# arnaucube/go-snark-study

Hardware: AMD Instinct MI355X
Metric: Groth16 constraints/sec (prove) at 2^20 R1CS (higher is better)
Workload: dtype u32 (9x29-bit Montgomery limbs of the 254-bit BN128 fields)

## Files before the change

### go-snark-study_amd/csrc/msm.h

```cpp
#pragma once
#include <algorithm>
#include <vector>

#include "ec.h"
#include "runtime.h"
#include "tables.h"

namespace gs {

struct PlanBuffers {
  DevBuf digits, hist, totals, offsets, entries, tiles, total;
  DevBuf chunk_bucket, heavy_list, counters;
  DevBuf recs, parts;
};

struct MsmPlan {
  uint32_t n = 0;
  int c = 0, W = 0;
  uint32_t B = 0;
  bool table_free = false;
  uint32_t nbuckets = 0;
  uint32_t chunk = 32;
  uint32_t maxchunks = 0;
  const uint32_t* offsets = nullptr;
  const uint32_t* entries = nullptr;
  const uint32_t* chunk_bucket = nullptr;
  const uint32_t* heavy_list = nullptr;
  const uint32_t* heavy_count = nullptr;
};

constexpr int kMaxWindowBits = 20;
int choose_window_bits(uint32_t n, int forced);
constexpr int kMinFreeWindowBits = 9, kMaxFreeWindowBits = 16;
int choose_window_bits_free(uint32_t n, int forced);

struct MsmBase {
  const BaseTable* table;
  size_t off;
  const uint32_t* points = nullptr;
  size_t npoints = 0;
};

struct LaunchShape { int njobs; bool g2; };
void build_plan(Ctx& c, int slot, const uint32_t* scalars_dev, uint32_t n, MsmPlan& plan, const std::vector<LaunchShape>& users, int cbits = 0,
                bool table_free = false, const uint32_t* term_index = nullptr, uint32_t index_bias = 0);
bool plan_partitions_first(int cbits);
uint32_t finite_mask_dev(Ctx& c, const uint32_t* g1_pts, const uint32_t* g2_pts, uint32_t n, uint32_t* mask_dev);

struct MsmPending {
  int njobs = 0, L = 1, slot = 0, c = 0, W = 0;
  bool table_free = false;
  uint32_t nblk_window = 0;
  uint32_t nblk = 0, n = 0;
  bool g2 = false;
  bool folded = false;
  const void* pinned_slot = nullptr;
  size_t stats_off = 0;
  std::shared_ptr<PhaseTimer> tacc, tker, tred;
};
void msm_enqueue_g1(Ctx& c, const MsmPlan& plan, const std::vector<MsmBase>& bases, int ws_base, int slot, MsmPending& p, hipStream_t tail_stream = nullptr);
void msm_enqueue_g2(Ctx& c, const MsmPlan& plan, const std::vector<MsmBase>& bases, int ws_base, int slot, MsmPending& p, hipStream_t tail_stream = nullptr);
void msm_book_timing(Ctx& c, const MsmPending& p);
void msm_finish_g1(Ctx& c, const MsmPending& p, std::vector<G1Xyzz>& out);
void msm_finish_g2(Ctx& c, const MsmPending& p, std::vector<G2Xyzz>& out);
void msm_run_g1(Ctx& c, const MsmPlan& plan, const std::vector<MsmBase>& bases, std::vector<G1Xyzz>& out);
void msm_run_g2(Ctx& c, const MsmPlan& plan, const std::vector<MsmBase>& bases, std::vector<G2Xyzz>& out);

uint32_t jacobian_to_affine_g1(Ctx& c, const uint32_t* jac_dev, uint32_t n, uint32_t* out_dev, uint32_t* first_bad = nullptr);
uint32_t jacobian_to_affine_g2(Ctx& c, const uint32_t* jac_dev, uint32_t n, uint32_t* out_dev, uint32_t* first_bad = nullptr);
uint32_t upload_jacobian_g1(Ctx& c, const uint64_t* jac_host, uint32_t n, uint32_t* out_dev, uint32_t* first_bad = nullptr);
uint32_t upload_jacobian_g2(Ctx& c, const uint64_t* jac_host, uint32_t n, uint32_t* out_dev, uint32_t* first_bad = nullptr);
void affine_to_jacobian_std_g1(Ctx& c, const uint32_t* aff_dev, uint32_t n, uint32_t* out_dev);
void affine_to_jacobian_std_g2(Ctx& c, const uint32_t* aff_dev, uint32_t n, uint32_t* out_dev);
void fixed_base_g1(Ctx& c, const uint32_t* scalars_dev, uint32_t n, uint32_t* out_dev);
void fixed_base_g2(Ctx& c, const uint32_t* scalars_dev, uint32_t n, uint32_t* out_dev);

G1Affine g1_affine_from_jacobian_std(const uint64_t jac[12]);
G2Affine g2_affine_from_jacobian_std(const uint64_t jac[24]);
bool g1_to_affine_std(const G1Xyzz& p, uint64_t out[8]);
bool g2_to_affine_std(const G2Xyzz& p, uint64_t out[16]);
G1Xyzz g1_mul_scalar(const G1Xyzz& p, const uint64_t k[4]);
G2Xyzz g2_mul_scalar(const G2Xyzz& p, const uint64_t k[4]);
template <class T>
struct HostFixedBase {
  std::vector<Xyzz<T>> win;
  void build(const Affine<T>& p);
  Xyzz<T> mul(const uint64_t k[4]) const;
};
extern template struct HostFixedBase<FqTag>;
extern template struct HostFixedBase<Fq2Tag>;

void fr_canon_words(const uint64_t k[4], uint32_t out[8]);

}
```

### go-snark-study_amd/csrc/msm.hip

```cpp
#include "msm.h"
#include "hostcopy.h"

#include <algorithm>
#include <cmath>
#include <cstdlib>
#include <future>
#include <type_traits>

#include "msm_kernels.h"

namespace gs {

static_assert(sizeof(G1Xyzz) == PointIO<FqTag>::kXyzzWords * 4, "G1 XYZZ must be raw limbs");
static_assert(sizeof(G2Xyzz) == PointIO<Fq2Tag>::kXyzzWords * 4, "G2 XYZZ must be raw limbs");

int choose_window_bits(uint32_t n, int forced) {
  if (forced >= 8 && forced <= kMaxWindowBits) return forced;
  static const double per_bucket = dev_knob_f("GS_WINDOW_COST_BUCKET", 6.0, 0.0, 64.0);
  static const int auto_max = (int)dev_knob("GS_AUTO_MAX_C", 17, 8, kMaxWindowBits);
  int best = 8;
  double best_cost = 1e300;
  for (int c = 8; c <= std::min(kMaxWindowBits, std::max(8, auto_max)); ++c) {
    const int W = 254 / c + 1;
    const double cost = (double)n * W + per_bucket * (double)(1u << (c - 1));
    if (cost < best_cost) { best_cost = cost; best = c; }
  }
  return best;
}

int choose_window_bits_free(uint32_t n, int forced) {
  if (forced) return std::min(kMaxFreeWindowBits, std::max(kMinFreeWindowBits, forced));
  static const double per_bucket = dev_knob_f("GS_WINDOW_COST_BUCKET_FREE", 3.0, 0.0, 64.0);
  int best = kMinFreeWindowBits;
  double best_cost = 1e300;
  for (int c = kMinFreeWindowBits; c <= kMaxFreeWindowBits; ++c) {
    const int W = 254 / c + 1;
    const double cost = (double)W * ((double)n + per_bucket * (double)(1u << (c - 1)));
    if (cost < best_cost) { best_cost = cost; best = c; }
  }
  return best;
}

static void exclusive_scan(Ctx& c, PlanBuffers& pb, const uint32_t* in, uint32_t* out, uint32_t n) {
  const uint32_t ntiles = (n + kScanTile - 1) / kScanTile;
  pb.tiles.ensure((size_t)ntiles * 4);
  pb.total.ensure(4);
  hipLaunchKernelGGL(k_scan_tiles, dim3(ntiles), dim3(kScanBlock), 0, c.stream, in, out, pb.tiles.as<uint32_t>(), n);
  hipLaunchKernelGGL(k_scan_tile_sums, dim3(1), dim3(1024), 0, c.stream, pb.tiles.as<uint32_t>(), ntiles, pb.total.as<uint32_t>());
  hipLaunchKernelGGL(k_scan_add, dim3(ntiles), dim3(kScanBlock), 0, c.stream, out, pb.tiles.as<uint32_t>(), n);
}

struct MsmState {
  PlanBuffers plan_slots[3 * Ctx::kSlots];
  DevBuf upload_scratch;
  DevBuf upload_flag;
  bool lds_attr_set = false;
};
static MsmState& msm_state(Ctx& c) { return c.state<MsmState>(c.msm_state); }

static uint32_t choose_chunk(uint64_t entries, uint32_t nbuckets, const std::vector<LaunchShape>& users) {
  static const int forced = (int)dev_knob("GS_CHUNK", 0, 4, 1024, 4);
  if (forced >= 4 && forced % 4 == 0) return (uint32_t)forced;
  static const int forced_h = (int)dev_knob("GS_CHUNK_H", 0, 4, 1024, 4);
  if (forced_h && users.size() == 1 && users[0].njobs == 1 && !users[0].g2) return (uint32_t)forced_h;
  uint32_t chunk = entries >= (1ull << 27) ? 64u : entries >= (1ull << 23) ? 32u : 16u;
  while (chunk < 1024u && entries / std::max<uint32_t>(nbuckets, 1u) > 32ull * chunk) chunk *= 2;
  return chunk;
}

static uint32_t part_min_ranges() {
  static const uint32_t v = (uint32_t)dev_knob("GS_PART_MIN_R", 4, 2, 64);
  return v;
}
bool plan_partitions_first(int cbits) {
  if (cbits < 1) return false;
  return std::max<uint32_t>(1u, (1u << (cbits - 1)) >> kRangeLog) >= part_min_ranges();
}

uint32_t finite_mask_dev(Ctx& c, const uint32_t* g1_pts, const uint32_t* g2_pts, uint32_t n, uint32_t* mask_dev) {
  const size_t words = ((size_t)n + 31) / 32;
  GS_HIP(hipMemsetAsync(mask_dev, 0, std::max<size_t>(words, 1) * 4, c.stream));
  DevBuf cnt(4);
  GS_HIP(hipMemsetAsync(cnt.p, 0, 4, c.stream));
  if (n) hipLaunchKernelGGL(k_finite_mask, grid1(n), dim3(256), 0, c.stream, g1_pts, (uint32_t)PointIO<FqTag>::kAffineWords, g2_pts,
                            (uint32_t)PointIO<Fq2Tag>::kAffineWords, n, mask_dev, cnt.as<uint32_t>());
  GS_HIP(hipGetLastError());
  uint32_t host = 0;
  GS_HIP(hipMemcpyAsync(&host, cnt.p, 4, hipMemcpyDeviceToHost, c.stream));
  GS_HIP(hipStreamSynchronize(c.stream));
  return host;
}

void build_plan(Ctx& c, int slot, const uint32_t* scalars_dev, uint32_t n, MsmPlan& plan, const std::vector<LaunchShape>& users, int cbits,
                bool table_free, const uint32_t* term_index, uint32_t index_bias) {
  MsmState& ms = msm_state(c);
  PlanBuffers& pb = ms.plan_slots[slot % (3 * Ctx::kSlots)];
  plan.n = n;
  plan.table_free = table_free;
  plan.c = cbits ? cbits : (table_free ? choose_window_bits_free(n, c.window_bits) : choose_window_bits(n, c.window_bits));
  if (table_free && (plan.c < kMinFreeWindowBits || plan.c > kMaxFreeWindowBits))
    throw HipError{hipErrorInvalidValue, "table-free plan outside 9..16 window bits", __LINE__};
  plan.W = 254 / plan.c + 1;
  plan.B = 1u << (plan.c - 1);
  plan.nbuckets = table_free ? (uint32_t)plan.W * plan.B : plan.B;
  plan.chunk = choose_chunk((uint64_t)n * plan.W, plan.nbuckets, users);
  plan.maxchunks = (uint32_t)(((size_t)n * plan.W + plan.chunk - 1) / plan.chunk) + 1;
  const size_t ncount = (size_t)plan.nbuckets + 1;
  PlanParams pp{};
  pp.n = n; pp.c = plan.c; pp.W = plan.W; pp.B = plan.B;
  pp.R = std::max<uint32_t>(1u, plan.B >> kRangeLog);
  pp.tf = table_free ? 1u : 0u;
  {
    const uint32_t want = std::max<uint32_t>(1u, 256u / (plan.W * pp.R));
    const uint32_t by_size = std::max<uint32_t>(1u, (n + 16383u) / 16384u);
    const uint32_t by_mem = std::max<uint32_t>(1u, (uint32_t)((64ull << 20) / ((uint64_t)plan.B * plan.W * 4)));
    pp.S = std::max<uint32_t>(1u, std::min(std::min<uint32_t>(16u, std::max<uint32_t>(want, 1u)), std::min(by_size, by_mem)));
    if (pp.R == 1 && !table_free) pp.S = std::max<uint32_t>(1u, std::min<uint32_t>(16u, by_size));
  }
  pp.slice = (n + pp.S - 1) / pp.S;
  pp.stride = (n + 63u) & ~63u;
  const bool wide = plan_partitions_first(plan.c);
  if (wide && term_index) throw HipError{hipErrorInvalidValue, "plans over a term list cannot be sorted partition-first (plan_partitions_first)", __LINE__};
  const uint32_t nparts = (uint32_t)plan.W * pp.R;
  if (wide && nparts > kMaxParts) throw HipError{hipErrorInvalidValue, "too many (window, range) partitions", __LINE__};
  if (!wide) pb.digits.ensure((size_t)std::max<uint32_t>(pp.stride, 64u) * plan.W * sizeof(digit_t));
  else {
    pb.recs.ensure(std::max<size_t>((size_t)n * plan.W, 1) * 8);
    pb.parts.ensure((size_t)(3 * kMaxParts + 4) * 4);
  }
  pb.hist.ensure((size_t)plan.B * plan.W * pp.S * 4);
  pb.totals.ensure(ncount * 4);
  pb.offsets.ensure(ncount * 4);
  pb.entries.ensure(((size_t)plan.maxchunks + 1) * plan.chunk * 4);
  pb.chunk_bucket.ensure((size_t)plan.maxchunks * 4);
  pb.heavy_list.ensure((size_t)plan.nbuckets * 4);
  pb.counters.ensure(16);
  const size_t lds = (size_t)std::min<uint32_t>(plan.B, kRangeBuckets) * 4;
  static const int sort_block = (int)dev_knob("GS_SORT_BLOCK", kSortBlock, 64, kSortBlock, 64);
  if (!ms.lds_attr_set) {
    GS_HIP(hipFuncSetAttribute(reinterpret_cast<const void*>(k_hist), hipFuncAttributeMaxDynamicSharedMemorySize, 128 * 1024));
    GS_HIP(hipFuncSetAttribute(reinterpret_cast<const void*>(k_scatter), hipFuncAttributeMaxDynamicSharedMemorySize, 128 * 1024));
    GS_HIP(hipFuncSetAttribute(reinterpret_cast<const void*>(k_hist_part), hipFuncAttributeMaxDynamicSharedMemorySize, 128 * 1024));
    GS_HIP(hipFuncSetAttribute(reinterpret_cast<const void*>(k_scatter_part), hipFuncAttributeMaxDynamicSharedMemorySize, 128 * 1024));
    ms.lds_attr_set = true;
  }
  GS_HIP(hipMemsetAsync(pb.totals.as<uint32_t>() + plan.nbuckets, 0, 4, c.stream));
  GS_HIP(hipMemsetAsync(pb.counters.p, 0, 16, c.stream));
  uint32_t* part_count = pb.parts.as<uint32_t>();
  uint32_t* part_base = part_count ? part_count + kMaxParts : nullptr;
  uint32_t* part_cursor = part_count ? part_base + kMaxParts + 4 : nullptr;
  if (n > 0 && wide) {
    GS_HIP(hipMemsetAsync(part_count, 0, (size_t)nparts * 4, c.stream));
    hipLaunchKernelGGL(k_part_count, grid1(n, kPartBlock), dim3(kPartBlock), 0, c.stream, scalars_dev, pp, part_count);
    hipLaunchKernelGGL(k_part_scan, dim3(1), dim3(64), 0, c.stream, part_count, nparts, part_base, part_cursor);
    hipLaunchKernelGGL(k_part_scatter, grid1(n, kPartBlock * kPartPerThread), dim3(kPartBlock), 0, c.stream, scalars_dev, pp, part_base, part_cursor,
                       pb.recs.as<uint2>());
    hipLaunchKernelGGL(k_hist_part, dim3(8 * pp.S * ((nparts + 7) / 8)), dim3(sort_block), lds, c.stream, pb.recs.as<uint2>(), part_base, pp, pb.hist.as<uint32_t>());
    hipLaunchKernelGGL(k_colscan, grid1(plan.B), dim3(256), 0, c.stream, pb.hist.as<uint32_t>(), pp, pb.totals.as<uint32_t>());
  } else if (n > 0) {
    hipLaunchKernelGGL(k_digits, grid1(n), dim3(256), 0, c.stream, scalars_dev, pp, pb.digits.as<digit_t>(), term_index, index_bias);
    hipLaunchKernelGGL(k_hist, dim3(plan.W, pp.S, pp.R), dim3(sort_block), lds, c.stream, pb.digits.as<digit_t>(), pp, pb.hist.as<uint32_t>());
    if (table_free) hipLaunchKernelGGL(k_colscan_windows, grid1(plan.nbuckets), dim3(256), 0, c.stream, pb.hist.as<uint32_t>(), pp, pb.totals.as<uint32_t>());
    else hipLaunchKernelGGL(k_colscan, grid1(plan.B), dim3(256), 0, c.stream, pb.hist.as<uint32_t>(), pp, pb.totals.as<uint32_t>());
  } else {
    GS_HIP(hipMemsetAsync(pb.totals.p, 0, ncount * 4, c.stream));
  }
  exclusive_scan(c, pb, pb.totals.as<uint32_t>(), pb.offsets.as<uint32_t>(), (uint32_t)ncount);
  if (n > 0) {
    if (wide) hipLaunchKernelGGL(k_scatter_part, dim3(8 * pp.S * ((nparts + 7) / 8)), dim3(sort_block), lds, c.stream, pb.recs.as<uint2>(), part_base, pp,
                                 pb.hist.as<uint32_t>(), pb.offsets.as<uint32_t>(), pb.entries.as<uint32_t>());
    else hipLaunchKernelGGL(k_scatter, dim3(plan.W, pp.S, pp.R), dim3(sort_block), lds, c.stream, pb.digits.as<digit_t>(), pp, pb.hist.as<uint32_t>(),
                            pb.offsets.as<uint32_t>(), pb.entries.as<uint32_t>(), term_index, index_bias);
    hipLaunchKernelGGL(k_chunk_map, grid1(plan.nbuckets), dim3(256), 0, c.stream, pb.offsets.as<uint32_t>(), plan.nbuckets, plan.chunk,
                       pb.chunk_bucket.as<uint32_t>(), pb.heavy_list.as<uint32_t>(), pb.counters.as<uint32_t>());
  }
  GS_HIP(hipGetLastError());
  plan.offsets = pb.offsets.as<uint32_t>();
  plan.entries = pb.entries.as<uint32_t>();
  plan.chunk_bucket = pb.chunk_bucket.as<uint32_t>();
  plan.heavy_list = pb.heavy_list.as<uint32_t>();
  plan.heavy_count = pb.counters.as<uint32_t>();
}

template <class T>
static void msm_enqueue(Ctx& c, const MsmPlan& plan, const std::vector<MsmBase>& bases, int ws_base, int slot, MsmPending& p,
                        hipStream_t tail_stream) {
  const int njobs = (int)bases.size();
  p = MsmPending{};
  p.njobs = njobs; p.slot = slot; p.n = plan.n; p.g2 = PointIO<T>::kAffineWords == 32;
  p.c = plan.c; p.W = plan.W;
  if (njobs == 0 || plan.n == 0) { p.njobs = plan.n == 0 ? -njobs : 0; return; }
  if (njobs > kMaxJobs) throw HipError{hipErrorInvalidValue, "too many MSM jobs", __LINE__};
  constexpr size_t pw = PointIO<T>::kXyzzWords;
  constexpr size_t aw = PointIO<T>::kAffineWords;
  static const uint32_t fold_env = (uint32_t)dev_knob("GS_FOLD_MAX", 0, 1, 256);
  const uint32_t fold_max = fold_env ? fold_env : (plan.n >= (1u << 19) ? 32u : 16u);
  static const uint32_t l_min = (uint32_t)dev_knob("GS_REDUCE_L", 4, 1, 32, 1, true);
  int L = (int)std::max<uint32_t>(1u, std::min<uint32_t>(l_min, plan.B / kReduceBlock));
  while (L < 32 && plan.B / ((uint32_t)kReduceBlock * (uint32_t)L) > fold_max) L *= 2;
  uint32_t nblk = (plan.B + kReduceBlock * L - 1) / (kReduceBlock * L);
  if (plan.table_free) {
    L = (int)std::max<uint32_t>(1u, std::min<uint32_t>(16u, plan.B / kReduceBlock));
    p.nblk_window = plan.B / ((uint32_t)kReduceBlock * (uint32_t)L);
    nblk = p.nblk_window * (uint32_t)plan.W;
    p.table_free = true;
  }
  p.L = L; p.nblk = nblk;
  p.folded = !plan.table_free && nblk > fold_max;
  if (p.folded && nblk > (uint32_t)kReduceBlock) throw HipError{hipErrorInvalidValue, "too many reduce workgroups for one fold", __LINE__};
  const size_t pair_bytes = (size_t)njobs * nblk * 2 * pw * 4, final_bytes = (size_t)njobs * pw * 4, stats_bytes = 16;
  const size_t out_bytes = (p.folded ? final_bytes : pair_bytes + final_bytes) + stats_bytes;
  if (out_bytes > Ctx::kPinnedBytes) throw HipError{hipErrorInvalidValue, "MSM result staging too small", __LINE__};
  p.stats_off = out_bytes - stats_bytes;
  AccJobs jobs{};
  DevBuf& outb = c.ws_out[ws_base % Ctx::kWsSets];
  outb.ensure(pair_bytes + final_bytes + stats_bytes);
  uint32_t* finals = outb.as<uint32_t>() + pair_bytes / 4;
  uint32_t* stats = finals + final_bytes / 4;
  for (int j = 0; j < njobs; ++j) {
    const BaseTable* t = bases[j].table;
    const uint32_t* points = nullptr;
    uint32_t row_stride = 0;
    if (plan.table_free) {
      if (!bases[j].points || bases[j].off + plan.n > bases[j].npoints)
        throw HipError{hipErrorInvalidValue, "MSM base array does not cover the plan", __LINE__};
      points = bases[j].points + bases[j].off * aw;
    } else {
      if (!t || t->c != plan.c || !t->rows.p || bases[j].off + plan.n > t->n)
        throw HipError{hipErrorInvalidValue, "MSM base table does not match the plan", __LINE__};
      points = t->rows.as<uint32_t>() + bases[j].off * aw;
      row_stride = (uint32_t)t->n;
    }
    DevBuf& bk = c.ws_buckets[(ws_base + j) % Ctx::kWsSets];
    DevBuf& mg = c.ws_chunks[(ws_base + j) % Ctx::kWsSets];
    DevBuf& pt = c.ws_partials[(ws_base + j) % Ctx::kWsSets];
    bk.ensure((size_t)plan.nbuckets * pw * 4);
    mg.ensure((size_t)plan.nbuckets * pw * 4);
    pt.ensure((size_t)plan.maxchunks * 2 * pw * 4);
    jobs.j[j] = AccJob{points, row_stride, bk.as<uint32_t>(), pt.as<uint32_t>(),
                       pt.as<uint32_t>() + (size_t)plan.maxchunks * pw, mg.as<uint32_t>(),
                       outb.as<uint32_t>() + (size_t)j * nblk * 2 * pw, finals + (size_t)j * pw};
  }
  p.tacc = std::make_shared<PhaseTimer>(c.stream);
  p.tker = std::make_shared<PhaseTimer>(c.stream);
  hipLaunchKernelGGL(k_bucket_accumulate<T>, dim3((plan.maxchunks + kAccBlock - 1) / kAccBlock, njobs), dim3(kAccBlock), 0, c.stream,
                     jobs, plan.offsets, plan.entries, plan.chunk_bucket, plan.nbuckets, plan.chunk);
  p.tker->stop();
  p.tacc->stop();
  hipStream_t ts = tail_stream ? tail_stream : c.stream;
  if (ts != c.stream) {
    hipEvent_t ev;
    GS_HIP(hipEventCreateWithFlags(&ev, hipEventDisableTiming));
    GS_HIP(hipEventRecord(ev, c.stream));
    GS_HIP(hipStreamWaitEvent(ts, ev, 0));
    GS_HIP(hipEventDestroy(ev));
  }
  p.tred = std::make_shared<PhaseTimer>(ts);
  static const long alone_below_log2 = dev_knob("GS_TAIL_ALONE_LOG2", 19, 0, 32);
  const bool alone = plan.n < (1ull << alone_below_log2);
  auto launch_tails = [&](auto alone_tag) {
    constexpr bool kAlone = decltype(alone_tag)::value;
    hipLaunchKernelGGL((k_heavy_combine<T, kAlone>), dim3(64, njobs), dim3(kHeavyBlock), 0, ts,
                       jobs, plan.offsets, plan.heavy_list, plan.heavy_count, plan.chunk);
    hipLaunchKernelGGL((k_heavy_finish<T, kAlone>), dim3(16, njobs), dim3(kHeavyBlock), 0, ts,
// ... 226 lines not shown
```

### go-snark-study_amd/csrc/msm_kernels.h

```cpp
#pragma once
#include <hip/hip_runtime.h>
#include <stdint.h>

#include "ec.h"
#include "point_io.h"

namespace gs {

struct PlanParams {
  uint32_t n;
  int c;
  int W;
  uint32_t B;
  uint32_t S;
  uint32_t slice;
  uint32_t stride;
  uint32_t R;
  uint32_t tf;
};
constexpr uint32_t kRangeLog = 15;
constexpr uint32_t kRangeBuckets = 1u << kRangeLog;

GS_HD int32_t next_digit(const uint32_t (&k)[8], const PlanParams& pp, int w, uint32_t& carry) {
  uint32_t raw = scalar_bits(k, w * pp.c, pp.c) + carry;
  if (raw > pp.B) { carry = 1; return (int32_t)raw - (int32_t)(2u * pp.B); }
  carry = 0;
  return (int32_t)raw;
}

using digit_t = uint32_t;
__global__ void __launch_bounds__(256) k_digits(const uint32_t* __restrict__ scalars, PlanParams pp, digit_t* __restrict__ digits,
                                                 const uint32_t* __restrict__ term_index, uint32_t index_bias) {
  wave_priority<GS_PRIO_PLAN>();
  const uint32_t i = blockIdx.x * blockDim.x + threadIdx.x;
  if (i >= pp.n) return;
  const uint32_t src = term_index ? term_index[i] - index_bias : i;
  uint32_t k[8];
  const uint4* s4 = reinterpret_cast<const uint4*>(scalars + (size_t)src * 8);
  uint4 lo = s4[0], hi = s4[1];
  k[0] = lo.x; k[1] = lo.y; k[2] = lo.z; k[3] = lo.w; k[4] = hi.x; k[5] = hi.y; k[6] = hi.z; k[7] = hi.w;
  scalar_canon(k);
  uint32_t carry = 0;
  for (int w = 0; w < pp.W; ++w) {
    const int32_t d = next_digit(k, pp, w, carry);
    digits[(size_t)w * pp.stride + i] = (digit_t)(d + (int32_t)pp.B - 1);
  }
}

__global__ void __launch_bounds__(256) k_finite_mask(const uint32_t* __restrict__ a, uint32_t wa, const uint32_t* __restrict__ b, uint32_t wb, uint32_t n,
                                                      uint32_t* __restrict__ mask, uint32_t* __restrict__ count) {
  const uint32_t i = blockIdx.x * blockDim.x + threadIdx.x;
  bool finite = false;
  if (i < n) {
    uint32_t acc = 0;
    if (a) for (uint32_t k = 0; k < wa; ++k) acc |= a[(size_t)i * wa + k];
    if (b) for (uint32_t k = 0; k < wb; ++k) acc |= b[(size_t)i * wb + k];
    finite = acc != 0;
  }
  if (finite) { atomicOr(&mask[i >> 5], 1u << (i & 31u)); atomicAdd(count, 1u); }
}

constexpr int kSortBlock = 1024;

__global__ void __launch_bounds__(kSortBlock) k_hist(const digit_t* __restrict__ digits, PlanParams pp, uint32_t* __restrict__ hist) {
  wave_priority<GS_PRIO_PLAN>();
  extern __shared__ uint32_t sh[];
  const uint32_t w = blockIdx.x, s = blockIdx.y, r = blockIdx.z;
  const uint32_t nb = min(pp.B, kRangeBuckets), base = r << kRangeLog;
  for (uint32_t b = threadIdx.x; b < nb; b += blockDim.x) sh[b] = 0;
  __syncthreads();
  const uint32_t lo = s * pp.slice, hi = min(pp.n, lo + pp.slice);
  const digit_t* row = digits + (size_t)w * pp.stride;
  const int32_t zero = (int32_t)pp.B - 1;
  for (uint32_t i = lo + threadIdx.x; i < hi; i += blockDim.x) {
    const int32_t d = (int32_t)row[i] - zero;
    if (d != 0) {
      const uint32_t b = (uint32_t)(d < 0 ? -d : d) - 1u;
      if ((b >> kRangeLog) == r) atomicAdd(&sh[b - base], 1u);
    }
  }
  __syncthreads();
  uint32_t* out = hist + ((size_t)w * pp.S + s) * pp.B + base;
  for (uint32_t b = threadIdx.x; b < nb; b += blockDim.x) out[b] = sh[b];
}

__global__ void __launch_bounds__(256) k_colscan(uint32_t* __restrict__ hist, PlanParams pp, uint32_t* __restrict__ totals) {
  wave_priority<GS_PRIO_PLAN>();
  const uint32_t b = blockIdx.x * blockDim.x + threadIdx.x;
  if (b >= pp.B) return;
  uint32_t* col = hist + b;
  const uint32_t nq = (uint32_t)pp.W * pp.S;
  uint32_t run = 0;
  for (uint32_t q = 0; q < nq; ++q) { const uint32_t t = col[(size_t)q * pp.B]; col[(size_t)q * pp.B] = run; run += t; }
  totals[b] = run;
}

__global__ void __launch_bounds__(256) k_colscan_windows(uint32_t* __restrict__ hist, PlanParams pp, uint32_t* __restrict__ totals) {
  wave_priority<GS_PRIO_PLAN>();
  const uint32_t i = blockIdx.x * blockDim.x + threadIdx.x;
  if (i >= (uint32_t)pp.W * pp.B) return;
  const uint32_t w = i / pp.B, b = i % pp.B;
  uint32_t* col = hist + (size_t)w * pp.S * pp.B + b;
  uint32_t run = 0;
  for (uint32_t q = 0; q < pp.S; ++q) { const uint32_t t = col[(size_t)q * pp.B]; col[(size_t)q * pp.B] = run; run += t; }
  totals[i] = run;
}

__global__ void __launch_bounds__(kSortBlock) k_scatter(const digit_t* __restrict__ digits, PlanParams pp, const uint32_t* __restrict__ hist,
                                                         const uint32_t* __restrict__ offsets, uint32_t* __restrict__ entries,
                                                         const uint32_t* __restrict__ term_index, uint32_t index_bias) {
  wave_priority<GS_PRIO_PLAN>();
  extern __shared__ uint32_t sh[];
  const uint32_t w = blockIdx.x, s = blockIdx.y, r = blockIdx.z;
  const uint32_t nb = min(pp.B, kRangeBuckets), base = r << kRangeLog;
  const uint32_t* pre = hist + ((size_t)w * pp.S + s) * pp.B + base;
  const uint32_t* off = offsets + (pp.tf ? (size_t)w * pp.B : (size_t)0);
  for (uint32_t b = threadIdx.x; b < nb; b += blockDim.x) sh[b] = off[base + b] + pre[b];
  __syncthreads();
  const uint32_t lo = s * pp.slice, hi = min(pp.n, lo + pp.slice);
  const digit_t* row = digits + (size_t)w * pp.stride;
  const int32_t zero = (int32_t)pp.B - 1;
  for (uint32_t i = lo + threadIdx.x; i < hi; i += blockDim.x) {
    const int32_t d = (int32_t)row[i] - zero;
    if (d != 0) {
      const uint32_t b = (uint32_t)(d < 0 ? -d : d) - 1u;
      if ((b >> kRangeLog) == r) {
        const uint32_t pos = atomicAdd(&sh[b - base], 1u);
        const uint32_t id = term_index ? term_index[i] - index_bias : i;
        entries[pos] = id | (w << kWindowShift) | (d < 0 ? kSignBit : 0u);
      }
    }
  }
}

constexpr int kPartBlock = 256;
constexpr int kPartPerThread = 4;
constexpr uint32_t kMaxParts = 512;

GS_HD void load_scalar_canon(const uint32_t* __restrict__ scalars, uint32_t i, uint32_t (&k)[8]) {
  const uint4* s4 = reinterpret_cast<const uint4*>(scalars + (size_t)i * 8);
  const uint4 lo = s4[0], hi = s4[1];
  k[0] = lo.x; k[1] = lo.y; k[2] = lo.z; k[3] = lo.w; k[4] = hi.x; k[5] = hi.y; k[6] = hi.z; k[7] = hi.w;
  scalar_canon(k);
}

__global__ void __launch_bounds__(kPartBlock) k_part_count(const uint32_t* __restrict__ scalars, PlanParams pp, uint32_t* __restrict__ part_count) {
  wave_priority<GS_PRIO_PLAN>();
  __shared__ uint32_t cnt[kMaxParts];
  const uint32_t nparts = (uint32_t)pp.W * pp.R;
  for (uint32_t t = threadIdx.x; t < nparts; t += kPartBlock) cnt[t] = 0;
  __syncthreads();
  const uint32_t i = blockIdx.x * kPartBlock + threadIdx.x;
  if (i < pp.n) {
    uint32_t k[8];
    load_scalar_canon(scalars, i, k);
    uint32_t carry = 0;
    for (int w = 0; w < pp.W; ++w) {
      const int32_t d = next_digit(k, pp, w, carry);
      if (d != 0) atomicAdd(&cnt[(uint32_t)w * pp.R + (((uint32_t)(d < 0 ? -d : d) - 1u) >> kRangeLog)], 1u);
    }
  }
  __syncthreads();
  for (uint32_t t = threadIdx.x; t < nparts; t += kPartBlock) if (cnt[t]) atomicAdd(&part_count[t], cnt[t]);
}

__global__ void __launch_bounds__(64) k_part_scan(uint32_t* __restrict__ part_count, uint32_t nparts, uint32_t* __restrict__ part_base,
                                                    uint32_t* __restrict__ part_cursor) {
  wave_priority<GS_PRIO_PLAN>();
  if (blockIdx.x != 0 || threadIdx.x != 0) return;
  uint32_t run = 0;
  for (uint32_t t = 0; t < nparts; ++t) { part_base[t] = run; run += part_count[t]; part_cursor[t] = 0; part_count[t] = 0; }
  part_base[nparts] = run;
}

__global__ void __launch_bounds__(kPartBlock) k_part_scatter(const uint32_t* __restrict__ scalars, PlanParams pp, const uint32_t* __restrict__ part_base,
                                                              uint32_t* __restrict__ part_cursor, uint2* __restrict__ recs) {
  wave_priority<GS_PRIO_PLAN>();
  __shared__ uint32_t cnt[kMaxParts];
  const uint32_t nparts = (uint32_t)pp.W * pp.R;
  for (uint32_t t = threadIdx.x; t < nparts; t += kPartBlock) cnt[t] = 0;
  __syncthreads();
  const uint32_t first = blockIdx.x * (kPartBlock * kPartPerThread);
  for (int j = 0; j < kPartPerThread; ++j) {
    const uint32_t i = first + j * kPartBlock + threadIdx.x;
    if (i >= pp.n) break;
    uint32_t k[8];
    load_scalar_canon(scalars, i, k);
    uint32_t carry = 0;
    for (int w = 0; w < pp.W; ++w) {
      const int32_t d = next_digit(k, pp, w, carry);
      if (d != 0) atomicAdd(&cnt[(uint32_t)w * pp.R + (((uint32_t)(d < 0 ? -d : d) - 1u) >> kRangeLog)], 1u);
    }
  }
  __syncthreads();
  for (uint32_t t = threadIdx.x; t < nparts; t += kPartBlock) {
    const uint32_t mine = cnt[t];
    cnt[t] = part_base[t] + (mine ? atomicAdd(&part_cursor[t], mine) : 0u);
  }
  __syncthreads();
  for (int j = 0; j < kPartPerThread; ++j) {
    const uint32_t i = first + j * kPartBlock + threadIdx.x;
    if (i >= pp.n) break;
    uint32_t k[8];
    load_scalar_canon(scalars, i, k);
    uint32_t carry = 0;
    for (int w = 0; w < pp.W; ++w) {
      const int32_t d = next_digit(k, pp, w, carry);
      if (d != 0) {
        const uint32_t b = (uint32_t)(d < 0 ? -d : d) - 1u;
        const uint32_t pos = atomicAdd(&cnt[(uint32_t)w * pp.R + (b >> kRangeLog)], 1u);
        recs[pos] = make_uint2(i | (d < 0 ? kSignBit : 0u), b);
      }
    }
  }
}

GS_HD bool part_of_block(uint32_t id, const PlanParams& pp, uint32_t& w, uint32_t& r, uint32_t& s) {
  const uint32_t xcd = id & 7u, j = id >> 3;
  const uint32_t p = xcd + 8u * (j / pp.S);
  s = j % pp.S;
// ... 33 lines not shown
  uint32_t w, r, s;
  if (!part_of_block(blockIdx.x, pp, w, r, s)) return;
  const uint32_t base = r << kRangeLog;
  const uint32_t* pre = hist + ((size_t)w * pp.S + s) * pp.B + base;
  for (uint32_t b = threadIdx.x; b < kRangeBuckets; b += blockDim.x) sh[b] = offsets[base + b] + pre[b];
  __syncthreads();
  uint32_t lo, hi;
  part_slice(part_base, pp, w, r, s, lo, hi);
  for (uint32_t e = lo + threadIdx.x; e < hi; e += blockDim.x) {
    const uint2 rec = recs[e];
    entries[atomicAdd(&sh[rec.y - base], 1u)] = rec.x | (w << kWindowShift);
  }
}

constexpr int kScanBlock = 256;
constexpr int kScanPerThread = 8;
constexpr int kScanTile = kScanBlock * kScanPerThread;

__global__ void __launch_bounds__(kScanBlock) k_scan_tiles(const uint32_t* __restrict__ in, uint32_t* __restrict__ out,
                                                            uint32_t* __restrict__ tile_sums, uint32_t n) {
  wave_priority<GS_PRIO_PLAN>();
  __shared__ uint32_t sh[kScanBlock];
  const uint32_t base = blockIdx.x * kScanTile + threadIdx.x * kScanPerThread;
  uint32_t v[kScanPerThread], sum = 0;
#pragma unroll
  for (int j = 0; j < kScanPerThread; ++j) { v[j] = (base + j < n) ? in[base + j] : 0u; sum += v[j]; }
  sh[threadIdx.x] = sum;
  __syncthreads();
  for (int off = 1; off < kScanBlock; off <<= 1) {
    uint32_t t = (threadIdx.x >= (uint32_t)off) ? sh[threadIdx.x - off] : 0u;
    __syncthreads();
    sh[threadIdx.x] += t;
    __syncthreads();
  }
  uint32_t run = sh[threadIdx.x] - sum;
#pragma unroll
  for (int j = 0; j < kScanPerThread; ++j) { if (base + j < n) out[base + j] = run; run += v[j]; }
  if (threadIdx.x == kScanBlock - 1) tile_sums[blockIdx.x] = sh[threadIdx.x];
}

__global__ void __launch_bounds__(1024) k_scan_tile_sums(uint32_t* __restrict__ tile_sums, uint32_t ntiles, uint32_t* __restrict__ total) {
  wave_priority<GS_PRIO_PLAN>();
  __shared__ uint32_t sh[1024];
  const uint32_t per = (ntiles + 1023u) / 1024u;
  const uint32_t b0 = threadIdx.x * per;
  uint32_t sum = 0;
  for (uint32_t j = 0; j < per; ++j) if (b0 + j < ntiles) sum += tile_sums[b0 + j];
  sh[threadIdx.x] = sum;
  __syncthreads();
  for (int off = 1; off < 1024; off <<= 1) {
    uint32_t t = (threadIdx.x >= (uint32_t)off) ? sh[threadIdx.x - off] : 0u;
    __syncthreads();
    sh[threadIdx.x] += t;
    __syncthreads();
  }
  uint32_t run = sh[threadIdx.x] - sum;
  for (uint32_t j = 0; j < per; ++j) if (b0 + j < ntiles) { uint32_t t = tile_sums[b0 + j]; tile_sums[b0 + j] = run; run += t; }
  if (threadIdx.x == 1023) *total = sh[1023];
}

__global__ void __launch_bounds__(kScanBlock) k_scan_add(uint32_t* __restrict__ out, const uint32_t* __restrict__ tile_sums, uint32_t n) {
  wave_priority<GS_PRIO_PLAN>();
  const uint32_t base = blockIdx.x * kScanTile + threadIdx.x * kScanPerThread;
  const uint32_t add = tile_sums[blockIdx.x];
#pragma unroll
  for (int j = 0; j < kScanPerThread; ++j) if (base + j < n) out[base + j] += add;
}

constexpr uint32_t kHeavySpan = 64;

__global__ void __launch_bounds__(256) k_chunk_map(const uint32_t* __restrict__ offsets, uint32_t nbuckets, uint32_t chunk,
                                                    uint32_t* __restrict__ chunk_bucket, uint32_t* __restrict__ heavy_list,
                                                    uint32_t* __restrict__ heavy_count) {
  wave_priority<GS_PRIO_PLAN>();
  const uint32_t b = blockIdx.x * blockDim.x + threadIdx.x;
  if (b >= nbuckets) return;
  const uint32_t o0 = offsets[b], o1 = offsets[b + 1];
  if (o1 == o0) return;
  const uint32_t t0 = (o0 + chunk - 1) / chunk, t1 = (o1 + chunk - 1) / chunk;
  for (uint32_t t = t0; t < t1; ++t) chunk_bucket[t] = b;
  if ((o1 - 1) / chunk - o0 / chunk > kHeavySpan) {
    heavy_list[atomicAdd(heavy_count, 1u)] = b;
  }
}

struct AccJob {
  const uint32_t* table;
  uint32_t row_stride;
  uint32_t* buckets;
  uint32_t* heads;
  uint32_t* tails;
  uint32_t* merged;
  uint32_t* out;
  uint32_t* final_out;
};
constexpr int kMaxJobs = 8;
struct AccJobs { AccJob j[kMaxJobs]; };

template <class T> struct AccTuning;
#ifndef GS_G1_WAVES
#define GS_G1_WAVES 3
#endif
#ifndef GS_G1_PREFETCH
#define GS_G1_PREFETCH 1
#endif
#ifndef GS_G2_TOUCH
#define GS_G2_TOUCH 0
#endif
template <> struct AccTuning<FqTag> { static constexpr int kMinWaves = GS_G1_WAVES; static constexpr bool kRegisterPrefetch = GS_G1_PREFETCH != 0; static constexpr bool kTouch = true; };
#ifndef GS_G2_WAVES
#define GS_G2_WAVES 2
#endif
#ifndef GS_G2_PREFETCH
#define GS_G2_PREFETCH 0
#endif
template <> struct AccTuning<Fq2Tag> { static constexpr int kMinWaves = GS_G2_WAVES; static constexpr bool kRegisterPrefetch = GS_G2_PREFETCH != 0; static constexpr bool kTouch = GS_G2_TOUCH != 0; };

#ifndef GS_ACC_BLOCK
#define GS_ACC_BLOCK 256
#endif
constexpr int kAccBlock = GS_ACC_BLOCK;
template <class T>
__global__ void __launch_bounds__(kAccBlock, AccTuning<T>::kMinWaves) k_bucket_accumulate(AccJobs jobs, const uint32_t* __restrict__ offsets,
                                                            const uint32_t* __restrict__ entries,
                                                            const uint32_t* __restrict__ chunk_bucket, uint32_t nbuckets, uint32_t chunk) {
  constexpr int pw = PointIO<T>::kXyzzWords;
  constexpr int aw = PointIO<T>::kAffineWords;
  const uint32_t t = blockIdx.x * blockDim.x + threadIdx.x;
  const uint32_t total = offsets[nbuckets];
  const uint32_t beg = t * chunk;
  if (beg >= total) return;
  const uint32_t end = min(beg + chunk, total);
  const AccJob job = jobs.j[blockIdx.y];
  uint32_t b = chunk_bucket[t];
  uint32_t bend = offsets[b + 1];
  bool started_before = offsets[b] < beg;
  constexpr bool kTight = GS_PAIR != 0 && T::kWords != 8;
  using Acc = std::conditional_t<kTight, XyzzAcc<T>, Xyzz<T>>;
  auto acc_inf = [] { if constexpr (kTight) return xyzz_acc_inf<T>(); else return xyzz_inf<T>(); };
  auto acc_store = [](uint32_t* p, const Acc& a) { if constexpr (kTight) store_xyzz<T>(p, to_xyzz(a)); else store_xyzz<T>(p, a); };
  Acc acc = acc_inf();
  const uint4* e4 = reinterpret_cast<const uint4*>(entries + beg);
  constexpr bool kPre = AccTuning<T>::kRegisterPrefetch;
  uint4 q = e4[0];
  uint32_t v = q.x;
  uint32_t nb = b;
  const uint32_t* np = job.table + ((size_t)((v >> kWindowShift) & 31u) * job.row_stride + (v & kIndexMask)) * aw;
  RawAffine<T> nextp;
  uint32_t touch = 0;
  if constexpr (kPre) nextp = load_raw_affine<T>(np);
  for (uint32_t e = beg; e < end; ++e) {
    const uint32_t cur = v;
    const uint32_t* cp = np;
    RawAffine<T> curp;
    if constexpr (kPre) curp = nextp;
    if (e >= bend) {
      acc_store((started_before ? job.heads + (size_t)t * pw : job.buckets + (size_t)b * pw), acc);
      started_before = false;
      acc = acc_inf();
      b = nb; bend = offsets[b + 1];
    }
    if (e + 1 < end) {
      const uint32_t k = (e + 1 - beg) & 3u;
      if (k == 0) q = e4[(e + 1 - beg) >> 2];
      v = k == 0 ? q.x : k == 1 ? q.y : k == 2 ? q.z : q.w;
      uint32_t nbend = offsets[nb + 1];
// ... 313 lines not shown
```

Baseline: 128.9 million.

## Add packed partition-first bucket sort for MSM plans at mid window sizes

Adds a third plan-building path for window sizes 15-17 with up to 2^22 terms. Scalars are counted and scattered into (range, window) partitions as packed 32-bit records (sign, low bucket bits, term index). Per-slice histograms, a column scan and a final scatter then produce the bucket-sorted entries. This replaces the digit-matrix path for these sizes to cut the memory traffic of writing and re-reading a full digit matrix. The cost is more kernel launches, recomputing digits twice, and a larger shared partition table (kMaxParts raised to 2048).

```diff
diff --git a/go-snark-study_amd/csrc/msm.h b/go-snark-study_amd/csrc/msm.h
--- a/go-snark-study_amd/csrc/msm.h
+++ b/go-snark-study_amd/csrc/msm.h
@@ -12,6 +12,7 @@
   DevBuf digits, hist, totals, offsets, entries, tiles, total;
   DevBuf chunk_bucket, heavy_list, counters;
   DevBuf recs, parts;
+  DevBuf pack_tables;
 };
 
 struct MsmPlan {
diff --git a/go-snark-study_amd/csrc/msm.hip b/go-snark-study_amd/csrc/msm.hip
--- a/go-snark-study_amd/csrc/msm.hip
+++ b/go-snark-study_amd/csrc/msm.hip
@@ -68,14 +68,19 @@
   return chunk;
 }
 
+enum class PlanSort { kMatrix, kWide, kPacked };
+constexpr uint32_t kPackedMinTerms = 1;
 static uint32_t part_min_ranges() {
   static const uint32_t v = (uint32_t)dev_knob("GS_PART_MIN_R", 4, 2, 64);
   return v;
 }
-bool plan_partitions_first(int cbits) {
-  if (cbits < 1) return false;
-  return std::max<uint32_t>(1u, (1u << (cbits - 1)) >> kRangeLog) >= part_min_ranges();
-}
+static PlanSort plan_sort(int cbits, uint32_t n, bool table_free, bool term_list) {
+  if (cbits < 1) return PlanSort::kMatrix;
+  if (std::max<uint32_t>(1u, (1u << (cbits - 1)) >> kRangeLog) >= part_min_ranges()) return PlanSort::kWide;
+  if (!table_free && !term_list && n >= kPackedMinTerms && pack_serves(n, cbits)) return PlanSort::kPacked;
+  return PlanSort::kMatrix;
+}
+bool plan_partitions_first(int cbits) { return plan_sort(cbits, 0, false, true) != PlanSort::kMatrix; }
 
 uint32_t finite_mask_dev(Ctx& c, const uint32_t* g1_pts, const uint32_t* g2_pts, uint32_t n, uint32_t* mask_dev) {
   const size_t words = ((size_t)n + 31) / 32;
@@ -89,6 +94,52 @@
   GS_HIP(hipMemcpyAsync(&host, cnt.p, 4, hipMemcpyDeviceToHost, c.stream));
   GS_HIP(hipStreamSynchronize(c.stream));
   return host;
+}
+
+static void publish_plan(MsmPlan& plan, PlanBuffers& pb) {
+  plan.offsets = pb.offsets.as<uint32_t>();
+  plan.entries = pb.entries.as<uint32_t>();
+  plan.chunk_bucket = pb.chunk_bucket.as<uint32_t>();
+  plan.heavy_list = pb.heavy_list.as<uint32_t>();
+  plan.heavy_count = pb.counters.as<uint32_t>();
+}
+
+static void build_plan_packed(Ctx& c, PlanBuffers& pb, const uint32_t* scalars_dev, MsmPlan& plan) {
+  PackParams P{};
+  P.n = plan.n; P.c = plan.c; P.W = plan.W; P.B = plan.B; P.chunk = plan.chunk;
+  P.L = pack_layout(plan.n, plan.c);
+  if (P.L.nparts > kMaxParts || P.L.NR > kPackMaxRanges || P.L.rb < (uint32_t)kPackMinRangeBits || (P.L.NR << P.L.rb) != plan.B)
+    throw HipError{hipErrorInvalidValue, "packed plan layout out of range", __LINE__};
+  const size_t nrec = (size_t)plan.n * plan.W;
+  pb.recs.ensure(nrec * 4);
+  const size_t table_words = 3 * (size_t)kMaxParts + 4 + 2 * (size_t)kPackMaxRanges + 4 + 8;
+  pb.pack_tables.ensure(table_words * 4);
+  pb.hist.ensure(((size_t)P.L.max_slices + 1) << P.L.rb << 2);
+  pb.offsets.ensure(((size_t)plan.nbuckets + 1) * 4);
+  pb.entries.ensure(((size_t)plan.maxchunks + 1) * plan.chunk * 4);
+  pb.chunk_bucket.ensure((size_t)plan.maxchunks * 4);
+  pb.heavy_list.ensure((size_t)plan.nbuckets * 4);
+  pb.counters.ensure(16);
+  PackTables T{};
+  T.count = pb.pack_tables.as<uint32_t>();
+  T.base = T.count + kMaxParts;
+  T.cursor = T.base + kMaxParts + 4;
+  T.xfirst = T.cursor + kMaxParts;
+  T.sbase = T.xfirst + kPackMaxRanges;
+  T.xtotal = T.sbase + kPackMaxRanges + 4;
+  GS_HIP(hipMemsetAsync(T.count, 0, (size_t)P.L.nparts * 4, c.stream));
+  GS_HIP(hipMemsetAsync(pb.counters.p, 0, 16, c.stream));
+  const uint32_t tiles = (plan.n + P.L.tile - 1) / P.L.tile, slice_grid = 8u * P.L.max_xslices;
+  hipLaunchKernelGGL(k_pack_count, dim3(tiles), dim3(kPackBlock), 0, c.stream, scalars_dev, P, T);
+  hipLaunchKernelGGL(k_pack_scan, dim3(1), dim3(kPackBlock), 0, c.stream, P, T);
+  hipLaunchKernelGGL(k_pack_scatter, dim3(tiles), dim3(kPackBlock), 0, c.stream, scalars_dev, P, T, pb.recs.as<uint32_t>());
+  hipLaunchKernelGGL(k_pack_hist, dim3(slice_grid), dim3(kPackBlock), 0, c.stream, pb.recs.as<uint32_t>(), P, T, pb.hist.as<uint32_t>());
+  hipLaunchKernelGGL(k_pack_offsets, dim3(P.L.NR), dim3(1u << P.L.rb), 0, c.stream, P, T, pb.hist.as<uint32_t>(), pb.offsets.as<uint32_t>(),
+                     pb.chunk_bucket.as<uint32_t>(), pb.heavy_list.as<uint32_t>(), pb.counters.as<uint32_t>());
+  hipLaunchKernelGGL(k_pack_entries, dim3(slice_grid), dim3(kPackBlock), 0, c.stream, pb.recs.as<uint32_t>(), P, T, pb.hist.as<uint32_t>(),
+                     pb.offsets.as<uint32_t>(), pb.entries.as<uint32_t>());
+  GS_HIP(hipGetLastError());
+  publish_plan(plan, pb);
 }
 
 void build_plan(Ctx& c, int slot, const uint32_t* scalars_dev, uint32_t n, MsmPlan& plan, const std::vector<LaunchShape>& users, int cbits,
@@ -119,7 +170,9 @@
   }
   pp.slice = (n + pp.S - 1) / pp.S;
   pp.stride = (n + 63u) & ~63u;
-  const bool wide = plan_partitions_first(plan.c);
+  const PlanSort sort = plan_sort(plan.c, n, table_free, term_index != nullptr);
+  if (sort == PlanSort::kPacked) { build_plan_packed(c, pb, scalars_dev, plan); return; }
+  const bool wide = sort == PlanSort::kWide;
   if (wide && term_index) throw HipError{hipErrorInvalidValue, "plans over a term list cannot be sorted partition-first (plan_partitions_first)", __LINE__};
   const uint32_t nparts = (uint32_t)plan.W * pp.R;
   if (wide && nparts > kMaxParts) throw HipError{hipErrorInvalidValue, "too many (window, range) partitions", __LINE__};
@@ -175,11 +228,7 @@
                        pb.chunk_bucket.as<uint32_t>(), pb.heavy_list.as<uint32_t>(), pb.counters.as<uint32_t>());
   }
   GS_HIP(hipGetLastError());
-  plan.offsets = pb.offsets.as<uint32_t>();
-  plan.entries = pb.entries.as<uint32_t>();
-  plan.chunk_bucket = pb.chunk_bucket.as<uint32_t>();
-  plan.heavy_list = pb.heavy_list.as<uint32_t>();
-  plan.heavy_count = pb.counters.as<uint32_t>();
+  publish_plan(plan, pb);
 }
 
 template <class T>
diff --git a/go-snark-study_amd/csrc/msm_kernels.h b/go-snark-study_amd/csrc/msm_kernels.h
--- a/go-snark-study_amd/csrc/msm_kernels.h
+++ b/go-snark-study_amd/csrc/msm_kernels.h
@@ -3,6 +3,7 @@
 #include <stdint.h>
 
 #include "ec.h"
+#include "plan_layout.h"
 #include "point_io.h"
 
 namespace gs {
@@ -21,12 +22,13 @@
 constexpr uint32_t kRangeLog = 15;
 constexpr uint32_t kRangeBuckets = 1u << kRangeLog;
 
-GS_HD int32_t next_digit(const uint32_t (&k)[8], const PlanParams& pp, int w, uint32_t& carry) {
-  uint32_t raw = scalar_bits(k, w * pp.c, pp.c) + carry;
-  if (raw > pp.B) { carry = 1; return (int32_t)raw - (int32_t)(2u * pp.B); }
+GS_HD int32_t digit_of(const uint32_t (&k)[8], int c, uint32_t B, int w, uint32_t& carry) {
+  uint32_t raw = scalar_bits(k, w * c, c) + carry;
+  if (raw > B) { carry = 1; return (int32_t)raw - (int32_t)(2u * B); }
   carry = 0;
   return (int32_t)raw;
 }
+GS_HD int32_t next_digit(const uint32_t (&k)[8], const PlanParams& pp, int w, uint32_t& carry) { return digit_of(k, pp.c, pp.B, w, carry); }
 
 using digit_t = uint32_t;
 __global__ void __launch_bounds__(256) k_digits(const uint32_t* __restrict__ scalars, PlanParams pp, digit_t* __restrict__ digits,
@@ -135,7 +137,7 @@
 
 constexpr int kPartBlock = 256;
 constexpr int kPartPerThread = 4;
-constexpr uint32_t kMaxParts = 512;
+constexpr uint32_t kMaxParts = 2048;
 
 GS_HD void load_scalar_canon(const uint32_t* __restrict__ scalars, uint32_t i, uint32_t (&k)[8]) {
   const uint4* s4 = reinterpret_cast<const uint4*>(scalars + (size_t)i * 8);
@@ -335,6 +337,214 @@
   if ((o1 - 1) / chunk - o0 / chunk > kHeavySpan) {
     heavy_list[atomicAdd(heavy_count, 1u)] = b;
   }
+}
+
+constexpr int kPackBlock = 256;
+struct PackParams {
+  uint32_t n;
+  int c, W;
+  uint32_t B;
+  uint32_t chunk;
+  PackLayout L;
+};
+struct PackTables {
+  uint32_t* count;
+  uint32_t* base;
+  uint32_t* cursor;
+  uint32_t* xfirst;
+  uint32_t* sbase;
+  uint32_t* xtotal;
+};
+
+__device__ __forceinline__ void pack_count_tile(const uint32_t* __restrict__ scalars, const PackParams& P, uint32_t* cnt) {
+  const uint32_t first = blockIdx.x * P.L.tile;
+  for (uint32_t j = 0; j < P.L.tile; j += kPackBlock) {
+    const uint32_t i = first + j + threadIdx.x;
+    if (i >= P.n) break;
+    uint32_t k[8];
+    load_scalar_canon(scalars, i, k);
+    uint32_t carry = 0;
+    for (int w = 0; w < P.W; ++w) {
+      const int32_t d = digit_of(k, P.c, P.B, w, carry);
+      if (d != 0) atomicAdd(&cnt[pack_partition(pack_bucket_range((uint32_t)(d < 0 ? -d : d) - 1u, P.L.rb), (uint32_t)w, (uint32_t)P.W)], 1u);
+    }
+  }
+}
+
+__global__ void __launch_bounds__(kPackBlock) k_pack_count(const uint32_t* __restrict__ scalars, PackParams P, PackTables T) {
+  wave_priority<GS_PRIO_PLAN>();
+  __shared__ uint32_t cnt[kMaxParts];
+  for (uint32_t t = threadIdx.x; t < P.L.nparts; t += kPackBlock) cnt[t] = 0;
+  __syncthreads();
+  pack_count_tile(scalars, P, cnt);
+  __syncthreads();
+  for (uint32_t t = threadIdx.x; t < P.L.nparts; t += kPackBlock) if (cnt[t]) atomicAdd(&T.count[t], cnt[t]);
+}
+
+__global__ void __launch_bounds__(kPackBlock) k_pack_scan(PackParams P, PackTables T) {
+  wave_priority<GS_PRIO_PLAN>();
+  static_assert(kMaxParts <= 8 * kPackBlock, "k_pack_scan: eight partitions per thread");
+  __shared__ uint32_t sb[kMaxParts + 1];
+  __shared__ uint32_t ssum[kPackBlock];
+  __shared__ uint32_t snsl[kPackMaxRanges];
+  const uint32_t nparts = P.L.nparts, per = (nparts + kPackBlock - 1u) / kPackBlock, t0 = threadIdx.x * per;
+  uint32_t v[8], sum = 0;
+#pragma unroll
+  for (uint32_t j = 0; j < 8; ++j) { v[j] = (j < per && t0 + j < nparts) ? T.count[t0 + j] : 0u; sum += v[j]; }
+  ssum[threadIdx.x] = sum;
+  __syncthreads();
+  for (int off = 1; off < kPackBlock; off <<= 1) {
+    const uint32_t t = (threadIdx.x >= (uint32_t)off) ? ssum[threadIdx.x - off] : 0u;
+    __syncthreads();
+    ssum[threadIdx.x] += t;
+    __syncthreads();
+  }
+  uint32_t run = ssum[threadIdx.x] - sum;
+#pragma unroll
+  for (uint32_t j = 0; j < 8; ++j)
+    if (j < per && t0 + j < nparts) { sb[t0 + j] = run; T.base[t0 + j] = run; T.cursor[t0 + j] = 0; run += v[j]; }
+  if (threadIdx.x == kPackBlock - 1) { sb[nparts] = ssum[kPackBlock - 1]; T.base[nparts] = ssum[kPackBlock - 1]; }
+  __syncthreads();
+  const uint32_t NR = P.L.NR, W = (uint32_t)P.W;
+  for (uint32_t r = threadIdx.x; r < NR; r += kPackBlock) snsl[r] = pack_slices(sb[(r + 1u) * W] - sb[r * W], P.L.slice_len);
+  __syncthreads();
+  for (uint32_t r = threadIdx.x; r < NR; r += kPackBlock) {
+    uint32_t xf = 0, sbv = 0;
+    for (uint32_t q = r & 7u; q < r; q += 8u) xf += snsl[q];
+    for (uint32_t q = 0; q < r; ++q) sbv += snsl[q];
+    T.xfirst[r] = xf;
+    T.sbase[r] = sbv;
+    if (r == NR - 1u) T.sbase[NR] = sbv + snsl[r];
+  }
+  if (threadIdx.x < 8u) {
+    uint32_t xt = 0;
+    for (uint32_t q = threadIdx.x; q < NR; q += 8u) xt += snsl[q];
+    T.xtotal[threadIdx.x] = xt;
+  }
+}
+
+__global__ void __launch_bounds__(kPackBlock) k_pack_scatter(const uint32_t* __restrict__ scalars, PackParams P, PackTables T, uint32_t* __restrict__ recs) {
+  wave_priority<GS_PRIO_PLAN>();
+  __shared__ uint32_t cnt[kMaxParts];
+  for (uint32_t t = threadIdx.x; t < P.L.nparts; t += kPackBlock) cnt[t] = 0;
+  __syncthreads();
+  pack_count_tile(scalars, P, cnt);
+  __syncthreads();
+  for (uint32_t t = threadIdx.x; t < P.L.nparts; t += kPackBlock) {
+    const uint32_t mine = cnt[t];
+    cnt[t] = T.base[t] + (mine ? atomicAdd(&T.cursor[t], mine) : 0u);
+  }
+  __syncthreads();
+  const uint32_t first = blockIdx.x * P.L.tile;
+  for (uint32_t j = 0; j < P.L.tile; j += kPackBlock) {
+    const uint32_t i = first + j + threadIdx.x;
+    if (i >= P.n) break;
+    uint32_t k[8];
+    load_scalar_canon(scalars, i, k);
+    uint32_t carry = 0;
+    for (int w = 0; w < P.W; ++w) {
+      const int32_t d = digit_of(k, P.c, P.B, w, carry);
+      if (d != 0) {
+        const uint32_t b = (uint32_t)(d < 0 ? -d : d) - 1u;
+        const uint32_t pos = atomicAdd(&cnt[pack_partition(pack_bucket_range(b, P.L.rb), (uint32_t)w, (uint32_t)P.W)], 1u);
+        recs[pos] = pack_record(d < 0, pack_bucket_low(b, P.L.rb), i, P.L.rb);
+      }
+    }
+  }
+}
+
+__device__ __forceinline__ bool pack_block_slice(const PackParams& P, const PackTables& T, uint32_t& r, uint32_t& row, uint32_t& lo, uint32_t& hi) {
+  const uint32_t x = blockIdx.x & 7u, j = blockIdx.x >> 3;
+  if (x >= P.L.NR || j >= T.xtotal[x]) return false;
+  r = x;
+  for (uint32_t q = x + 8u; q < P.L.NR && T.xfirst[q] <= j; q += 8u) r = q;
+  const uint32_t s = j - T.xfirst[r];
+  row = T.sbase[r] + s;
+  pack_slice_bounds(T.base[r * (uint32_t)P.W], T.base[(r + 1u) * (uint32_t)P.W], s, P.L.slice_len, lo, hi);
+  return true;
+}
+
+__global__ void __launch_bounds__(kPackBlock) k_pack_hist(const uint32_t* __restrict__ recs, PackParams P, PackTables T, uint32_t* __restrict__ hist) {
+  wave_priority<GS_PRIO_PLAN>();
+  __shared__ uint32_t sh[1u << kPackMaxRangeBits];
+  uint32_t r, row, lo, hi;
+  if (!pack_block_slice(P, T, r, row, lo, hi)) return;
+  const uint32_t rb = P.L.rb, nb = 1u << rb;
+  for (uint32_t b = threadIdx.x; b < nb; b += kPackBlock) sh[b] = 0;
+  __syncthreads();
+  uint32_t e = lo + threadIdx.x;
+  for (; e + 3u * kPackBlock < hi; e += 4u * kPackBlock) {
+    const uint32_t r0 = recs[e], r1 = recs[e + kPackBlock], r2 = recs[e + 2u * kPackBlock], r3 = recs[e + 3u * kPackBlock];
+    atomicAdd(&sh[record_bucket_low(r0, rb)], 1u);
+    atomicAdd(&sh[record_bucket_low(r1, rb)], 1u);
+    atomicAdd(&sh[record_bucket_low(r2, rb)], 1u);
+    atomicAdd(&sh[record_bucket_low(r3, rb)], 1u);
+  }
+  for (; e < hi; e += kPackBlock) atomicAdd(&sh[record_bucket_low(recs[e], rb)], 1u);
+  __syncthreads();
+  uint32_t* out = hist + (size_t)row * nb;
+  for (uint32_t b = threadIdx.x; b < nb; b += kPackBlock) out[b] = sh[b];
+}
+
+__global__ void __launch_bounds__(1 << kPackMaxRangeBits) k_pack_offsets(PackParams P, PackTables T, uint32_t* __restrict__ hist, uint32_t* __restrict__ offsets,
+                                                                         uint32_t* __restrict__ chunk_bucket, uint32_t* __restrict__ heavy_list,
+                                                                         uint32_t* __restrict__ heavy_count) {
+  wave_priority<GS_PRIO_PLAN>();
+  __shared__ uint32_t sc[1u << kPackMaxRangeBits];
+  const uint32_t r = blockIdx.x, b = threadIdx.x, nb = 1u << P.L.rb;
+  const uint32_t row0 = T.sbase[r], row1 = T.sbase[r + 1u];
+  uint32_t* col = hist + (size_t)row0 * nb + b;
+  uint32_t run = 0, row = row0;
+  for (; row + 4u <= row1; row += 4u, col += 4u * (size_t)nb) {
+    const uint32_t t0 = col[0], t1 = col[nb], t2 = col[2u * (size_t)nb], t3 = col[3u * (size_t)nb];
+    col[0] = run; col[nb] = run + t0; col[2u * (size_t)nb] = run + t0 + t1; col[3u * (size_t)nb] = run + t0 + t1 + t2;
+    run += t0 + t1 + t2 + t3;
+  }
+  for (; row < row1; ++row, col += nb) { const uint32_t t = col[0]; col[0] = run; run += t; }
+  sc[b] = run;
+  __syncthreads();
+  for (uint32_t off = 1; off < nb; off <<= 1) {
+    const uint32_t t = (b >= off) ? sc[b - off] : 0u;
+    __syncthreads();
+    sc[b] += t;
+    __syncthreads();
+  }
+  const uint32_t o0 = T.base[r * (uint32_t)P.W] + sc[b] - run, o1 = o0 + run;
+  const uint32_t bucket = pack_bucket_of(r, b, P.L.rb);
+  offsets[bucket] = o0;
+  if (bucket == P.B - 1u) offsets[P.B] = o1;
+  if (o1 == o0) return;
+  const uint32_t chunk = P.chunk;
+  const uint32_t c0 = (o0 + chunk - 1u) / chunk, c1 = (o1 + chunk - 1u) / chunk;
+  for (uint32_t t = c0; t < c1; ++t) chunk_bucket[t] = bucket;
+  if ((o1 - 1u) / chunk - o0 / chunk > kHeavySpan) heavy_list[atomicAdd(heavy_count, 1u)] = bucket;
+}
+
+__global__ void __launch_bounds__(kPackBlock) k_pack_entries(const uint32_t* __restrict__ recs, PackParams P, PackTables T, const uint32_t* __restrict__ hist,
+                                                              const uint32_t* __restrict__ offsets, uint32_t* __restrict__ entries) {
+  wave_priority<GS_PRIO_PLAN>();
+  __shared__ uint32_t sh[1u << kPackMaxRangeBits];
+  __shared__ uint32_t wb[32];
+  uint32_t r, row, lo, hi;
+  if (!pack_block_slice(P, T, r, row, lo, hi)) return;
+  const uint32_t rb = P.L.rb, nb = 1u << rb, W = (uint32_t)P.W;
+  const uint32_t* pre = hist + (size_t)row * nb;
+  const uint32_t* off = offsets + ((size_t)r << rb);
+  for (uint32_t b = threadIdx.x; b < nb; b += kPackBlock) sh[b] = off[b] + pre[b];
+  if (threadIdx.x <= W) wb[threadIdx.x] = T.base[r * W + threadIdx.x];
+  __syncthreads();
+  uint32_t w = 0;
+  auto put = [&](uint32_t e, uint32_t rec) {
+    while (w + 1u < W && e >= wb[w + 1u]) ++w;
+    const uint32_t pos = atomicAdd(&sh[record_bucket_low(rec, rb)], 1u);
+    entries[pos] = record_sign(rec) | (w << kWindowShift) | record_term(rec, rb);
+  };
+  uint32_t e = lo + threadIdx.x;
+  for (; e + 3u * kPackBlock < hi; e += 4u * kPackBlock) {
+    const uint32_t r0 = recs[e], r1 = recs[e + kPackBlock], r2 = recs[e + 2u * kPackBlock], r3 = recs[e + 3u * kPackBlock];
+    put(e, r0); put(e + kPackBlock, r1); put(e + 2u * kPackBlock, r2); put(e + 3u * kPackBlock, r3);
+  }
+  for (; e < hi; e += kPackBlock) put(e, recs[e]);
 }
 
 struct AccJob {
diff --git a/go-snark-study_amd/csrc/plan_layout.h b/go-snark-study_amd/csrc/plan_layout.h
--- /dev/null
+++ b/go-snark-study_amd/csrc/plan_layout.h
@@ -0,0 +1,84 @@
+#pragma once
+#include <stdint.h>
+#include <hip/hip_runtime.h>
+
+#ifndef GS_HD
+#define GS_HD __host__ __device__ __forceinline__
+#endif
+
+namespace gs {
+
+constexpr int kPackMaxRangeBits = 10;
+constexpr int kPackMinRangeBits = 9;
+constexpr int kPackMinWindowBits = 15, kPackMaxWindowBits = 17;
+constexpr uint32_t kPackMaxTerms = 1u << 22;
+constexpr uint32_t kPackMaxRanges = 1u << (kPackMaxWindowBits - 1 - kPackMinRangeBits);
+constexpr uint32_t kPackRecSign = 0x80000000u;
+
+GS_HD int pack_ceil_log2(uint32_t n) {
+  int k = 0;
+  while (k < 32 && ((uint64_t)1 << k) < n) ++k;
+  return k;
+}
+GS_HD int pack_range_bits(uint32_t n) {
+  const int room = 31 - pack_ceil_log2(n < 1u ? 1u : n);
+  return room < kPackMaxRangeBits ? room : kPackMaxRangeBits;
+}
+GS_HD bool pack_serves(uint32_t n, int c) {
+  return n >= 1u && n <= kPackMaxTerms && c >= kPackMinWindowBits && c <= kPackMaxWindowBits;
+}
+
+struct PackLayout {
+  uint32_t rb, tb;
+  uint32_t W;
+  uint32_t NR;
+  uint32_t nparts;
+  uint32_t tile;
+  uint32_t slice_len;
+  uint32_t max_xslices;
+  uint32_t max_slices;
+};
+
+GS_HD uint32_t pack_tile(uint32_t NR) { return 64u * NR < 1024u ? 1024u : 64u * NR; }
+GS_HD uint32_t pack_slice_len(uint32_t n, uint32_t W) {
+  const uint64_t want = ((uint64_t)n * W + 1023u) / 1024u;
+  uint32_t len = 2048u;
+  while (len < 16384u && len < want) len *= 2u;
+  return len;
+}
+GS_HD PackLayout pack_layout(uint32_t n, int c) {
+  PackLayout L;
+  L.rb = (uint32_t)pack_range_bits(n);
+  L.tb = 31u - L.rb;
+  L.W = (uint32_t)(254 / c + 1);
+  L.NR = (1u << (c - 1)) >> L.rb;
+  L.nparts = L.NR * L.W;
+  L.tile = pack_tile(L.NR);
+  L.slice_len = pack_slice_len(n, L.W);
+  const uint32_t by_len = (uint32_t)(((uint64_t)n * L.W + L.slice_len - 1u) / L.slice_len);
+  L.max_xslices = by_len + (L.NR + 7u) / 8u;
+  L.max_slices = by_len + L.NR;
+  return L;
+}
+
+GS_HD uint32_t pack_record(bool negative, uint32_t bucket_low, uint32_t term, uint32_t rb) {
+  return (negative ? kPackRecSign : 0u) | (bucket_low << (31u - rb)) | term;
+}
+GS_HD uint32_t record_sign(uint32_t rec) { return rec & kPackRecSign; }
+GS_HD uint32_t record_bucket_low(uint32_t rec, uint32_t rb) { return (rec >> (31u - rb)) & ((1u << rb) - 1u); }
+GS_HD uint32_t record_term(uint32_t rec, uint32_t rb) { return rec & ((1u << (31u - rb)) - 1u); }
+
+GS_HD uint32_t pack_bucket_range(uint32_t bucket, uint32_t rb) { return bucket >> rb; }
+GS_HD uint32_t pack_bucket_low(uint32_t bucket, uint32_t rb) { return bucket & ((1u << rb) - 1u); }
+GS_HD uint32_t pack_partition(uint32_t range, uint32_t window, uint32_t W) { return range * W + window; }
+GS_HD uint32_t pack_partition_range(uint32_t part, uint32_t W) { return part / W; }
+GS_HD uint32_t pack_partition_window(uint32_t part, uint32_t W) { return part % W; }
+GS_HD uint32_t pack_bucket_of(uint32_t range, uint32_t bucket_low, uint32_t rb) { return (range << rb) | bucket_low; }
+
+GS_HD uint32_t pack_slices(uint32_t len, uint32_t slice_len) { return (len + slice_len - 1u) / slice_len; }
+GS_HD void pack_slice_bounds(uint32_t p0, uint32_t p1, uint32_t s, uint32_t slice_len, uint32_t& lo, uint32_t& hi) {
+  lo = p0 + s * slice_len;
+  hi = p1 - lo < slice_len ? p1 : lo + slice_len;
+}
+
+}
```

Measured after the change: 123.1 million. -4.5%, worse.
